# raulmur/ORB_SLAM

Measured on AMD Instinct MI355X. Metric: frames/s ORB extract+match @640x480, 1000 kp, higher is better.
Workload: dtype u8; 1 GPU; vga: 640x480 grayscale stream, 8 levels, nFeatures 1000, S-blocks frames, extract + Hamming top-2 match vs previous frame (BASELINE.json configs[1] + the frame-to-frame match of the metric); resident_frames_per_gpu=2048, lanes=4, parity_checked_frames=0, parity_mismatches=0, library_build_id=15f67f48a050b108, lane_placement=2

## Files before the change

orb_slam_amd/csrc/k_fast.hip:

```cpp
#include <algorithm>
#include <type_traits>

#include "orbx_device.h"
#include "orbx_launch.h"
#include "k_blur_strip.h"

namespace orbx {

__device__ __forceinline__ int fast_pair_test(const uint8_t* c, int S, int v, int t) {
    const int x0 = c[3 * S], x1 = c[3 * S + 1], x2 = c[2 * S + 2], x3 = c[S + 3], x4 = c[3], x5 = c[-S + 3], x6 = c[-2 * S + 2], x7 = c[-3 * S + 1];
    const int x8 = c[-3 * S], x9 = c[-3 * S - 1], x10 = c[-2 * S - 2], x11 = c[-S - 3], x12 = c[-3], x13 = c[S - 3], x14 = c[2 * S - 2], x15 = c[3 * S - 1];
    const int a = imax3(imax3(imin(x0, x8), imin(x1, x9), imin(x2, x10)), imax3(imin(x3, x11), imin(x4, x12), imin(x5, x13)), imax(imin(x6, x14), imin(x7, x15)));
    const int bq = imin3(imin3(imax(x0, x8), imax(x1, x9), imax(x2, x10)), imin3(imax(x3, x11), imax(x4, x12), imax(x5, x13)), imin(imax(x6, x14), imax(x7, x15)));
    return (int)(v - a > t) | (int)(bq - v > t);
}

__device__ __forceinline__ int fast_score_raw(const uint8_t* c, int S, int v, int tmin) {
    int x[16];
    x[0] = c[3 * S]; x[1] = c[3 * S + 1]; x[2] = c[2 * S + 2]; x[3] = c[S + 3]; x[4] = c[3]; x[5] = c[-S + 3]; x[6] = c[-2 * S + 2]; x[7] = c[-3 * S + 1];
    x[8] = c[-3 * S]; x[9] = c[-3 * S - 1]; x[10] = c[-2 * S - 2]; x[11] = c[-S - 3]; x[12] = c[-3]; x[13] = c[S - 3]; x[14] = c[2 * S - 2]; x[15] = c[3 * S - 1];
    int hi3[16], lo3[16];
#pragma unroll
    for (int k = 0; k < 16; k++) {
        hi3[k] = imax3(x[k], x[(k + 1) & 15], x[(k + 2) & 15]);
        lo3[k] = imin3(x[k], x[(k + 1) & 15], x[(k + 2) & 15]);
    }
    int hi9[16], lo9[16];
#pragma unroll
    for (int k = 0; k < 16; k++) {
        hi9[k] = imax3(hi3[k], hi3[(k + 3) & 15], hi3[(k + 6) & 15]);
        lo9[k] = imin3(lo3[k], lo3[(k + 3) & 15], lo3[(k + 6) & 15]);
    }
    const int min_hi9 = imin3(imin3(imin3(hi9[0], hi9[1], hi9[2]), imin3(hi9[3], hi9[4], hi9[5]), imin3(hi9[6], hi9[7], hi9[8])),
                              imin3(imin3(hi9[9], hi9[10], hi9[11]), imin3(hi9[12], hi9[13], hi9[14]), hi9[15]), 255);
    const int max_lo9 = imax3(imax3(imax3(lo9[0], lo9[1], lo9[2]), imax3(lo9[3], lo9[4], lo9[5]), imax3(lo9[6], lo9[7], lo9[8])),
                              imax3(imax3(lo9[9], lo9[10], lo9[11]), imax3(lo9[12], lo9[13], lo9[14]), lo9[15]), 0);
    const int s = imax(v - min_hi9, max_lo9 - v) - 1;
    return s >= tmin ? s : 0;
}

struct FastHdr { int n_hi, n_lo, overflow, pad1; int wsum[8]; int pad2[4]; };
static_assert(sizeof(FastHdr) == 64, "LDS carve");

__device__ __forceinline__ int lane_rank(unsigned long long m) {
    return (int)__builtin_amdgcn_mbcnt_hi((unsigned)(m >> 32), __builtin_amdgcn_mbcnt_lo((unsigned)m, 0u));
}
template <bool ALIGNED, int NT, int PPT, bool GATHER = false>
__device__ __forceinline__ void fast_band_task(const Batch& b, int frame, int item, uint8_t* smem) {
    constexpr int NW = NT / 64;
    static_assert((NW & (NW - 1)) == 0, "wave roles rotate modulo NW");
    constexpr int Q0CAP = fast_q0cap(PPT), Q1CAP = FAST_Q1CAP, Q2CAP = FAST_Q2CAP, Q3CAP = FAST_Q3CAP;
    constexpr int WQ_BYTES = fast_wave_queue_bytes(PPT);
    const DevGeom& g = b.g;
    const BandGeom bg = b.bands[item];
    const int level = bg.level;
    const LevelGeom& L = g.lv[level];
    const int lane = threadIdx.x & 63, wave = ORBX_FAST_ROTATE ? (wave_id() + item) & (NW - 1) : wave_id(), tid = wave * 64 + lane;
    const int cw = bg.x1 - bg.x0 + 1, ch = bg.ey1 - bg.ey0 + 1;
    CellState* cst = b.cstate + (long long)frame * g.nbands_total + item;
    const int hint = b.fallback_hint ? (int)((uint32_t)cst->thr >> 8) : 0;
    if (cw <= 0 || ch <= 0) {
        if (tid == 0) { CellState st; st.n_all = 0; st.n_hi = 0; st.n_lo = 0; st.thr = g.tmin; *cst = st; }
        return;
    }
    const int own_lo = bg.y0 - bg.ey0, own_hi = bg.y1 - bg.ey0;
    const int gxb = (bg.x0 - 3) & ~3;
    const int xoff = (bg.x0 - 3) - gxb;
    const int nd = fast_row_dwords(xoff, cw);
    const int S = nd * 4;
    const int x_first = xoff + 3;
    const int nrows = ch + 6;
    FastHdr* hdr = reinterpret_cast<FastHdr*>(smem);
    unsigned long long* cmask = reinterpret_cast<unsigned long long*>(smem + sizeof(FastHdr));
    uint8_t* wq = smem + sizeof(FastHdr) + g.fast_max_chunks * 8 + wave * WQ_BYTES;
    uint32_t* q0 = reinterpret_cast<uint32_t*>(wq);
    uint16_t* q1 = reinterpret_cast<uint16_t*>(wq + Q0CAP * 4);
    uint16_t* q2 = q1 + Q1CAP;
    uint16_t* q3 = q2 + Q2CAP;
    uint8_t* s_img = smem + sizeof(FastHdr) + g.fast_max_chunks * 8 + NW * WQ_BYTES;
    uint8_t* s_sc = s_img + g.fast_max_img;
    const int q_own_lo = (3 + own_lo) * S, q_own_hi = (3 + own_hi + 1) * S;
    const int nchunks = (q_own_hi - q_own_lo + 63) >> 6;
    long long stride64;
    const uint8_t* src = plain_plane<GATHER>(b, L, level, frame, stride64);
    auto clear_lds = [&]() {
        for (int i = tid; i < ((nrows * S + 15) >> 4); i += NT) reinterpret_cast<uint4*>(s_sc)[i] = make_uint4(0, 0, 0, 0);
        if (tid < (int)(sizeof(FastHdr) / 4)) reinterpret_cast<int*>(hdr)[tid] = 0;
        for (int i = tid; i < nchunks; i += NT) cmask[i] = 0ull;
    };
    if (ALIGNED) {
        typedef const void __attribute__((address_space(1))) * gptr_t;
        typedef void __attribute__((address_space(3))) * lptr_t;
        const uint8_t* src0 = src + (long long)(bg.ey0 - 3) * stride64 + gxb;
        clear_lds();
        {
            const int cpr = nd >> 2, nchunks16 = nrows * cpr;
            const float inv_cpr = bg.inv_cpr;
            for (int q0 = 64 * wave; q0 < nchunks16; q0 += 64 * NW) {
                const int q = q0 + lane;
                int r, c;
                split_px(imin(q, nchunks16 - 1), cpr, inv_cpr, r, c);
                const uint8_t* ga = src0 + (long long)r * stride64 + 16 * c;
                if (q < nchunks16) __builtin_amdgcn_global_load_lds((gptr_t)ga, (lptr_t)(s_img + 16 * q0), 16, 0, 0);
            }
        }
        asm volatile("s_waitcnt vmcnt(0)" ::: "memory");
    } else {
        const int total = nrows * nd;
        const float inv_nd0 = bg.inv_nd;
        const uint8_t* src0 = src + (long long)(bg.ey0 - 3) * stride64 + gxb;
        const int xm = L.w - 1 - gxb;
        for (int i0 = 0; i0 < total; i0 += NT * 8) {
            uint32_t v4[8];
#pragma unroll
            for (int k = 0; k < 8; k++) {
                const int i = i0 + k * NT + tid;
                v4[k] = 0;
                if (i < total) {
                    int r, d;
                    split_px(i, nd, inv_nd0, r, d);
                    const uint8_t* row = src0 + (long long)r * stride64;
                    v4[k] = (uint32_t)row[imin(4 * d, xm)] | (uint32_t)row[imin(4 * d + 1, xm)] << 8 | (uint32_t)row[imin(4 * d + 2, xm)] << 16 |
                            (uint32_t)row[imin(4 * d + 3, xm)] << 24;
                }
            }
            if (i0 == 0) clear_lds();
#pragma unroll
            for (int k = 0; k < 8; k++) {
                const int i = i0 + k * NT + tid;
                if (i < total) reinterpret_cast<uint32_t*>(s_img)[i] = v4[k];
            }
        }
    }
    __syncthreads();

    constexpr int FAST_HINT_RUN = 6;
    int tmin = ORBX_FAST_TWO_PASS ? (hint >= FAST_HINT_RUN && g.fast_th > 7 ? 7 : g.fast_th) : g.tmin;
    const float inv_nd = bg.inv_nd;
    int n0 = 0, n1 = 0, n2 = 0, n3 = 0;

    auto score_vals = [&](bool on, int p) {
        int sc = 0;
        if (on) {
            const uint8_t* c = s_img + p;
            sc = fast_score_raw(c, S, c[0], tmin);
            s_sc[p] = (uint8_t)sc;
        }
        const unsigned long long mk = __ballot(sc != 0);
        if (mk) {
            const int add = __popcll(mk);
            if (n3 + add <= Q3CAP) { if (sc) q3[n3 + lane_rank(mk)] = (uint16_t)p; }
            n3 += add;
        }
    };
    auto score_step = [&](const uint16_t* q, int m) { score_vals(lane < m, lane < m ? (int)q[lane] : 0); };
    auto pair_step = [&](const uint16_t* q, int m) {
        int pass = 0, p = 0;
        if (lane < m) {
            p = q[lane];
            const uint8_t* c = s_img + p;
            pass = fast_pair_test(c, S, c[0], tmin);
        }
        const unsigned long long mk = __ballot(pass);
        if (mk) {
            if (pass) q2[n2 + lane_rank(mk)] = (uint16_t)p;
            n2 += __popcll(mk);
            if (n2 >= 64) { n2 -= 64; score_step(q2 + n2, 64); }
        }
    };
    auto expand_step = [&](const uint32_t* q, int m) {
        uint32_t e = 0;
        if (lane < m) e = q[lane];
        const int idx = (int)(e & 0x3FFFu);
        int r, d;
        split_px(idx, nd, inv_nd, r, d);
        const int col0 = 4 * d - x_first;
        const int f[4] = {(int)((e >> 15) & 1u) & (int)((unsigned)col0 < (unsigned)cw), (int)((e >> 14) & 1u) & (int)((unsigned)(col0 + 1) < (unsigned)cw),
                          (int)((e >> 31) & 1u) & (int)((unsigned)(col0 + 2) < (unsigned)cw), (int)((e >> 30) & 1u) & (int)((unsigned)(col0 + 3) < (unsigned)cw)};
#pragma unroll
        for (int j = 0; j < 4; j++) {
            const unsigned long long mk = __ballot(f[j]);
            if (mk) {
                if (f[j]) q1[n1 + lane_rank(mk)] = (uint16_t)(4 * idx + j);
                n1 += __popcll(mk);
            }
            if (j & 1) while (n1 >= 64) { n1 -= 64; pair_step(q1 + n1, 64); }
        }
    };

    const uint32_t M8 = 0x00FF00FFu, HH = 0x80008000u;
    uint32_t KD = (uint32_t)(0x8000 - tmin - 1) * 0x00010001u;
    auto compass4 = [&](uint32_t C, uint32_t E, uint32_t W, uint32_t Nn, uint32_t Ss) -> uint32_t {
        uint32_t P[2];
#pragma unroll
        for (int hlf = 0; hlf < 2; hlf++) {
            const uint32_t c = hlf ? (C >> 8) & M8 : C & M8, n = hlf ? (Nn >> 8) & M8 : Nn & M8, s = hlf ? (Ss >> 8) & M8 : Ss & M8,
                           e = hlf ? (E >> 8) & M8 : E & M8, w = hlf ? (W >> 8) & M8 : W & M8;
            const uint32_t vd = c + KD, vb = KD - c;
            const uint32_t dk = ((vd - n) | (vd - s)) & ((vd - e) | (vd - w));
            const uint32_t br = ((n + vb) | (s + vb)) & ((e + vb) | (w + vb));
            P[hlf] = dk | br;
        }
        return (P[0] & HH) | ((P[1] & HH) >> 1);
    };
    const int i_begin = 3 * nd, i_end = (ch + 3) * nd;
    constexpr int RG = NW * 64 * PPT;
    auto round = [&](auto full_c, int base) {
        constexpr bool FULL = decltype(full_c)::value;
        const int i0 = base + wave * 64 + lane;
        uint32_t C[PPT], E[PPT], W[PPT], Nn[PPT], Ss[PPT];
#pragma unroll
        for (int k = 0; k < PPT; k++) {
            const int ik = FULL ? i0 + k * NW * 64 : imin(i0 + k * NW * 64, i_end - 1);
            const uint8_t* pk = s_img + 4 * ik;
            C[k] = *reinterpret_cast<const uint32_t*>(pk);
            E[k] = __builtin_amdgcn_alignbyte(*reinterpret_cast<const uint32_t*>(pk + 4), C[k], 3);
            W[k] = __builtin_amdgcn_alignbyte(C[k], *reinterpret_cast<const uint32_t*>(pk - 4), 1);
            Nn[k] = *reinterpret_cast<const uint32_t*>(pk - 3 * S);
            Ss[k] = *reinterpret_cast<const uint32_t*>(pk + 3 * S);
        }
#pragma unroll
        for (int k = 0; k < PPT; k++) {
            const int i = i0 + k * NW * 64;
            uint32_t Q = compass4(C[k], E[k], W[k], Nn[k], Ss[k]);
            if (!FULL && i >= i_end) Q = 0;
            const unsigned long long mk = __ballot(Q != 0);
            if (mk) {
                if (Q) q0[n0 + lane_rank(mk)] = Q | (uint32_t)i;
                n0 += __popcll(mk);
                if (n0 >= 64) { n0 -= 64; expand_step(q0 + n0, 64); }
            }
        }
    };
    for (;;) {
    {
        int base = i_begin;
        for (; base + RG <= i_end; base += RG) round(std::true_type{}, base);
        if (base < i_end) round(std::false_type{}, base);
    }
    if (n0) expand_step(q0, n0);
    for (int base = 0; base < n1 + n2; base += 64) {
        const int i = base + lane;
        const bool on = i < n1 + n2;
        score_vals(on, on ? (int)(i < n1 ? q1[i] : q2[i - n1]) : 0);
    }
    if (n3 > Q3CAP && lane == 0) hdr->overflow = 1;
    __syncthreads();

    auto nms_test = [&](int p, int s) -> bool {
        const uint8_t* sp = s_sc + p;
        const int mx = imax3(imax3(sp[-1], sp[1], sp[-S]), imax3(sp[S], sp[-S - 1], sp[-S + 1]), imax(sp[S - 1], sp[S + 1]));
        if (s > mx) {
            const int bit = p - q_own_lo;
            atomicOr(&cmask[bit >> 6], 1ull << (bit & 63));
        }
        return s > mx;
    };
    auto nms_px = [&](int p, int s) {
        if (nms_test(p, s)) {
            if (s >= g.fast_th) atomicAdd(&hdr->n_hi, 1);
            if (s >= 7) atomicAdd(&hdr->n_lo, 1);
        }
    };
    if (!hdr->overflow) {
        int c_hi = 0, c_lo = 0;
        for (int i0 = 0; i0 < n3; i0 += 64) {
            const int i = i0 + lane;
            int s = 0;
            bool keep = false;
            if (i < n3) {
                const int p = q3[i];
                s = s_sc[p];
                keep = p >= q_own_lo && p < q_own_hi && nms_test(p, s);
            }
            c_hi += __popcll(__ballot(keep && s >= g.fast_th));
            c_lo += __popcll(__ballot(keep && s >= 7));
        }
        if (lane == 0 && (c_hi | c_lo)) { atomicAdd(&hdr->n_hi, c_hi); atomicAdd(&hdr->n_lo, c_lo); }
    } else {
        const int d_lo = q_own_lo >> 2, d_hi = q_own_hi >> 2;
        for (int i = d_lo + tid; i < d_hi; i += NT) {
            uint32_t sc4 = reinterpret_cast<const uint32_t*>(s_sc)[i];
            while (sc4) {
                const int j = (__ffs((int)sc4) - 1) >> 3;
                const int s = (int)((sc4 >> (8 * j)) & 255u);
                sc4 &= ~(255u << (8 * j));
                nms_px(4 * i + j, s);
            }
        }
    }
    __syncthreads();
    if (tmin <= 7 || __builtin_amdgcn_readfirstlane(hdr->n_hi) > 3) break;
    __syncthreads();
    clear_lds();
    tmin = 7;
    KD = (uint32_t)(0x8000 - 7 - 1) * 0x00010001u;
    n0 = n1 = n2 = n3 = 0;
    __syncthreads();
    }
    Cand* out = b.cand + (long long)frame * g.frame_cands + L.cand_base + bg.cand_off;
    const float inv_S = bg.inv_s;
    int run_base = 0;
    for (int c0 = 0; c0 < nchunks; c0 += NT) {
        const bool busy = c0 + 64 * wave < nchunks;
        unsigned long long m = 0ull;
        int cnt = 0, incl = 0;
        if (busy) {
            if (c0 + tid < nchunks) m = cmask[c0 + tid];
            cnt = __popcll(m);
            incl = wave_scan_inclusive(cnt);
        }
        if (NW > 1) {
            if (lane == 63) hdr->wsum[wave] = incl;
            __syncthreads();
        }
        int run = run_base + incl - cnt, total = NW > 1 ? 0 : __builtin_amdgcn_readlane(incl, 63);
        if (NW > 1 && busy) {
#pragma unroll
            for (int wv = 0; wv < NW; wv++) { const int t = hdr->wsum[wv]; if (wv < wave) run += t; total += t; }
        }
        while (m) {
            const int bit = __ffsll((long long)m) - 1;
            m &= m - 1;
            const int p = q_own_lo + (c0 + tid) * 64 + bit;
            int r, xr;
            split_px(p, S, inv_S, r, xr);
            Cand e;
            e.pos = (uint32_t)(bg.x0 + xr - x_first) | ((uint32_t)(bg.ey0 + r - 3) << 16);
            e.resp = (float)s_sc[p];
            out[run++] = e;
        }
        run_base += total;
        if (NW > 1 && c0 + NT < nchunks) __syncthreads();
    }
    if (tid == 0) {
        CellState st;
        st.n_all = run_base; st.n_hi = hdr->n_hi; st.n_lo = hdr->n_lo;
        st.thr = tmin | ((st.n_hi <= 3 && g.fast_th > 7 ? imin(hint + 1, FAST_HINT_RUN) : 0) << 8);
        *cst = st;
    }
}

template <bool ALIGNED, int NT, int PPT, bool GATHER>
__device__ __forceinline__ void k_fast_cells_body(const Batch& b) {
    extern __shared__ __attribute__((aligned(16))) uint8_t smem[];
    int frame, item;
    if (!frame_item_magic(b, blockIdx.x, (unsigned)b.g.nbands_total, b.g.nbands_magic, frame, item)) return;
    fast_band_task<ALIGNED, NT, PPT, GATHER>(b, frame, item, smem);
}
template <bool ALIGNED, int NT, int PPT>
__global__ __launch_bounds__(NT) void k_fast_cells(Batch b) { k_fast_cells_body<ALIGNED, NT, PPT, false>(b); }
template <bool ALIGNED, int NT, int PPT>
__global__ __launch_bounds__(NT) void k_fast_cells_gather(Batch b) { k_fast_cells_body<ALIGNED, NT, PPT, true>(b); }

template <bool ALIGNED, bool SMALL, bool GATHER>
__device__ __forceinline__ void k_fast_blur_body(const Batch& b) {
    extern __shared__ __attribute__((aligned(16))) uint8_t smem[];
    constexpr FastShape A = SMALL ? FAST_SMALL : FAST_LARGE;
    constexpr int NW = A.threads / 64;
    const DevGeom& g = b.g;
    const int nblur = (g.nbtiles_total_s + NW - 1) / NW;
    const int per_frame = nblur + g.nbands_total;
    const int frame = blockIdx.x / per_frame, item = blockIdx.x - frame * per_frame;
    if (item < nblur) {
        const int t = item * NW + wave_id();
        if (t < g.nbtiles_total_s) blur_strip<ALIGNED, BLUR_ROWS_SMALL, GATHER>(b, frame, t);
    } else fast_band_task<ALIGNED, A.threads, A.ppt, GATHER>(b, frame, item - nblur, smem);
}
template <bool ALIGNED, bool SMALL>
__global__ __launch_bounds__(SMALL ? FAST_SMALL.threads : FAST_LARGE.threads) void k_fast_blur(Batch b) { k_fast_blur_body<ALIGNED, SMALL, false>(b); }
template <bool ALIGNED, bool SMALL>
__global__ __launch_bounds__(SMALL ? FAST_SMALL.threads : FAST_LARGE.threads) void k_fast_blur_gather(Batch b) { k_fast_blur_body<ALIGNED, SMALL, true>(b); }


int launch_fast(const Batch& b, const HostGeom& hg, hipStream_t stream, bool fuse_blur) {
    const DevGeom& g = hg.g;
    const int F = b.nframes;
    const bool aligned = (level0_bits(b) & 3) == 0;
    const size_t lds = (size_t)g.fast_lds_bytes;
    auto launch = [&](auto kern, int threads) -> bool {
        if (lds > 64 * 1024 && hipFuncSetAttribute(reinterpret_cast<const void*>(kern), hipFuncAttributeMaxDynamicSharedMemorySize, (int)lds) != hipSuccess) return false;
        hipLaunchKernelGGL(kern, dim3(frame_item_blocks(b, g.nbands_total)), dim3(threads), lds, stream, b);
        return true;
    };
    constexpr FastShape A = FAST_SMALL, B = FAST_LARGE;
    bool ok;
    if (fuse_blur) {
        const int threads = g.fast_small ? A.threads : B.threads;
        const int per_frame = (g.nbtiles_total_s + threads / 64 - 1) / (threads / 64) + g.nbands_total;
        auto launch2 = [&](auto kern) -> bool {
            if (lds > 64 * 1024 && hipFuncSetAttribute(reinterpret_cast<const void*>(kern), hipFuncAttributeMaxDynamicSharedMemorySize, (int)lds) != hipSuccess) return false;
            hipLaunchKernelGGL(kern, dim3(F * per_frame), dim3(threads), lds, stream, b);
            return true;
        };
        if (b.img_tab) {
            if (g.fast_small) ok = aligned ? launch2(k_fast_blur_gather<true, true>) : launch2(k_fast_blur_gather<false, true>);
            else ok = aligned ? launch2(k_fast_blur_gather<true, false>) : launch2(k_fast_blur_gather<false, false>);
        } else if (g.fast_small) ok = aligned ? launch2(k_fast_blur<true, true>) : launch2(k_fast_blur<false, true>);
        else ok = aligned ? launch2(k_fast_blur<true, false>) : launch2(k_fast_blur<false, false>);
    } else if (b.img_tab) {
        if (g.fast_small) ok = aligned ? launch(k_fast_cells_gather<true, A.threads, A.ppt>, A.threads) : launch(k_fast_cells_gather<false, A.threads, A.ppt>, A.threads);
        else ok = aligned ? launch(k_fast_cells_gather<true, B.threads, B.ppt>, B.threads) : launch(k_fast_cells_gather<false, B.threads, B.ppt>, B.threads);
    } else if (g.fast_small) ok = aligned ? launch(k_fast_cells<true, A.threads, A.ppt>, A.threads) : launch(k_fast_cells<false, A.threads, A.ppt>, A.threads);
    else ok = aligned ? launch(k_fast_cells<true, B.threads, B.ppt>, B.threads) : launch(k_fast_cells<false, B.threads, B.ppt>, B.threads);
    if (!ok) return ORBX_ERR_DEVICE;
    ORBX_LAUNCH_CHECK();
    return ORBX_OK;
}

}
```

orb_slam_amd/csrc/orbx_geometry.hip:

```cpp
#include <cfloat>
#include <climits>
#include <cmath>
#include <cstdlib>
#include <cstring>

#include "orbx_internal.h"

namespace orbx {

static inline int round_even(double v) { return (int)std::lrint(v); }
static inline int floor_int(double v) { int i = (int)v; return i - (i > v); }
static inline int ceil_int(double v) { int i = (int)v; return i + (i < v); }
static inline int16_t sat16(float v) {
    int iv = round_even(v);
    return (int16_t)(iv < SHRT_MIN ? SHRT_MIN : iv > SHRT_MAX ? SHRT_MAX : iv);
}
static inline int align_up(int v, int a) { return (v + a - 1) / a * a; }

static int build_geometry_band(const orbx_params& p, int w, int h, HostGeom& out, std::string& err, const int band_px, const FastShape& shape) {
    const int threads = shape.threads;
    const int nl = p.nlevels;
    if (nl < 1 || nl > MAX_LEVELS) { err = "nlevels out of range [1,16]"; return ORBX_ERR_ARG; }
    if (p.nfeatures < 1) { err = "nfeatures must be >= 1"; return ORBX_ERR_ARG; }
    if (!(p.scale_factor > 1.0f) || p.scale_factor > 2.5f) { err = "scale_factor must be in (1, 2.5]"; return ORBX_ERR_ARG; }
// ... 138 lines not shown
                        bg.inv_nd = 1.0f / (float)nd;
                        bg.inv_s = 1.0f / (float)(nd * 4);
                        bg.inv_cpr = 1.0f / (float)(nd >> 2);
                    }
                    cand_off += bg.cand_cap;
                    c.cand_cap += bg.cand_cap;
                    c.nbands++;
                    out.bands.push_back(bg);
                }
                out.cells.push_back(c);
            }
        cell_base += L.ncells;
        cand_base += cand_off;
        L.sel_base = sel_base;
        L.sel_cap = std::min(cand_off, L.ncells * L.nfeat_cell + L.ncells * L.ncells + L.ndesired + 64);
        sel_base += L.sel_cap;
        L.slot_base = slot_base;
        slot_base += L.ndesired;
        L.quad_base = quad_base;
        quad_base += (L.ndesired + 3) / 4;

        L.btiles_x = (L.w + 247) / 248;
        L.btiles_y = (L.h + BLUR_ROWS - 1) / BLUR_ROWS;
        L.btile_base = btile_base;
        btile_base += L.btiles_x * L.btiles_y;
        L.btiles_y_s = (L.h + BLUR_ROWS_SMALL - 1) / BLUR_ROWS_SMALL;
        L.btile_base_s = btile_base_s;
        btile_base_s += L.btiles_x * L.btiles_y_s;
        {
            const int nsteps = (L.h + 31) / 32;
            L.mb_strips = (L.w + 32 * MB_TILES - 1) / (32 * MB_TILES);
            L.mb_bands = (nsteps + MB_BAND_STEPS - 1) / MB_BAND_STEPS;
            L.mb_band_steps = (nsteps + L.mb_bands - 1) / L.mb_bands;
            L.mb_n = L.mb_strips * L.mb_bands;
        }
        L.mb_base = mb_base;
        mb_base += L.mb_n;

        if (l > 0) {
            const int sw = g.lv[l - 1].w, sh = g.lv[l - 1].h, dw = L.w, dh = L.h;
            if (sw > 32767 || sh > 32767) { err = "image too large"; return ORBX_ERR_ARG; }
            const double inv_x = (double)dw / sw, inv_y = (double)dh / sh;
            const double scale_x = 1. / inv_x, scale_y = 1. / inv_y;
            L.tabx_off = (int)out.tabx.size();
            L.taby_off = (int)out.taby.size();
            for (int dx = 0; dx < dw; dx++) {
                float fx = (float)((dx + 0.5) * scale_x - 0.5);
                int sx = floor_int(fx);
                fx -= sx;
                if (sx < 0) { fx = 0; sx = 0; }
                if (sx >= sw - 1) { fx = 0; sx = sw - 1; }
                ResizeX e;
                e.sx = (int16_t)sx;
                e.sx1 = (int16_t)std::min(sx + 1, sw - 1);
                e.a0 = sat16((1.f - fx) * 2048);
                e.a1 = sat16(fx * 2048);
                out.tabx.push_back(e);
            }
            for (int dy = 0; dy < dh; dy++) {
                float fy = (float)((dy + 0.5) * scale_y - 0.5);
                int sy = floor_int(fy);
                fy -= sy;
                ResizeY e;
                e.sy0 = (int16_t)std::min(std::max(sy, 0), sh - 1);
                e.sy1 = (int16_t)std::min(std::max(sy + 1, 0), sh - 1);
                e.b0 = sat16((1.f - fy) * 2048);
                e.b1 = sat16(fy * 2048);
                out.taby.push_back(e);
            }
            {
                const ResizeX* tx = out.tabx.data() + L.tabx_off;
                const ResizeY* ty = out.taby.data() + L.taby_off;
                int nd_max = 1, nr_max = 1;
                for (int bx0 = 0; bx0 < dw; bx0 += 256) {
                    const int bx1 = std::min(bx0 + 255, dw - 1);
                    nd_max = std::max(nd_max, ((tx[bx1].sx1 - (tx[bx0].sx & ~3)) >> 2) + 1);
                }
                for (int by0 = 0; by0 < dh; by0 += RZ_ROWS) {
                    const int by1 = std::min(by0 + RZ_ROWS - 1, dh - 1);
                    nr_max = std::max(nr_max, ty[by1].sy1 - ty[by0].sy0 + 1);
                }
                L.rz_pitch = 4 * nd_max + 8;
                L.rz_rows = nr_max;
                int span = 1;
                for (int x0 = 0; x0 < dw; x0 += 4) span = std::max(span, tx[std::min(x0 + 3, dw - 1)].sx1 - tx[x0].sx + 1);
                L.rz_window = span <= 8 ? 1 : 0;
                if (L.rz_pitch * L.rz_rows > 64 * 1024) { err = "resize tile does not fit the LDS"; return ORBX_ERR_CAPACITY; }
            }
        }
    }
    {
        constexpr int tile[2] = {ORBX_PYR_TILE};
        g.npyr_groups = 0;
        out.pyr_tab.clear();
        bool ok = scaleFactor <= 2.0 && nl > 1 && !getenv("ORBX_PYR_PER_LEVEL");
        int l0 = 0;
        while (ok && l0 < nl - 1) {
            if (g.npyr_groups == PYR_MAX_GROUPS) { ok = false; break; }
            PyrGroup pg;
            memset(&pg, 0, sizeof(pg));
            pg.l0 = l0;
            constexpr int depth_cfg[2] = {ORBX_PYR_DEPTH};
            pg.depth = std::min(std::min(l0 == 0 ? depth_cfg[0] : depth_cfg[1], PYR_MAX_DEPTH), nl - 1 - l0);
            const LevelGeom& LD = g.lv[l0 + pg.depth];
            pg.ntx = (LD.w + tile[0] - 1) / tile[0];
            pg.nty = (LD.h + tile[1] - 1) / tile[1];
            auto chain = [&](int n, int tsz, bool is_x, std::vector<int>& tab) {
                const int base = (int)tab.size();
                tab.resize(base + (size_t)(pg.depth + 1) * (n + 1) * 2);
                auto at = [&](int k, int i, int e) -> int& { return tab[base + ((size_t)k * (n + 1) + i) * 2 + e]; };
                const int dim_d = is_x ? LD.w : LD.h;
                for (int i = 0; i <= n; i++) { at(pg.depth, i, 0) = std::min(i * tsz, dim_d); at(pg.depth, i, 1) = std::min((i + 1) * tsz, dim_d) - 1; }
                at(pg.depth, n, 1) = dim_d;
                for (int k = pg.depth; k >= 1; k--) {
                    const LevelGeom& Lk = g.lv[l0 + k];
                    const LevelGeom& Ls = g.lv[l0 + k - 1];
                    const int dk = is_x ? Lk.w : Lk.h, ds = is_x ? Ls.w : Ls.h;
                    for (int i = 0; i <= n; i++) {
                        const int s0 = at(k, i, 0);
                        int src = ds;
                        if (s0 < dk) src = is_x ? (out.tabx[Lk.tabx_off + s0].sx & ~3) : out.taby[Lk.taby_off + s0].sy0;
                        at(k - 1, i, 0) = src;
                    }
                    for (int i = 0; i < n; i++) {
                        const int e0 = std::min(at(k, i, 1), dk - 1);
                        int need = is_x ? out.tabx[Lk.tabx_off + e0].sx1 : out.taby[Lk.taby_off + e0].sy1;
                        need = std::max(need, at(k - 1, i + 1, 0) - 1);
                        if (is_x) need = std::min(need | 3, ds - 1);
                        at(k - 1, i, 1) = std::max(need, at(k - 1, i, 0));
                    }
                    at(k - 1, n, 1) = ds;
                }
                return base;
            };
            pg.xtab = chain(pg.ntx, tile[0], true, out.pyr_tab);
            pg.ytab = chain(pg.nty, tile[1], false, out.pyr_tab);
            int off = 0;
            for (int k = 0; k < pg.depth; k++) {
                int maxw = 4, maxh = 1;
                for (int i = 0; i < pg.ntx; i++) maxw = std::max(maxw, out.pyr_tab[pg.xtab + ((size_t)k * (pg.ntx + 1) + i) * 2 + 1] - out.pyr_tab[pg.xtab + ((size_t)k * (pg.ntx + 1) + i) * 2] + 1);
                for (int i = 0; i < pg.nty; i++) maxh = std::max(maxh, out.pyr_tab[pg.ytab + ((size_t)k * (pg.nty + 1) + i) * 2 + 1] - out.pyr_tab[pg.ytab + ((size_t)k * (pg.nty + 1) + i) * 2] + 1);
                pg.pitch[k] = align_up(maxw, 4) + 4;
                pg.lds_off[k] = off;
                off += align_up(pg.pitch[k] * maxh, 16);
            }
            pg.lds_bytes = off;
            if (off > 64 * 1024) { ok = false; break; }
            g.pyr[g.npyr_groups++] = pg;
            l0 += pg.depth;
        }
        if (!ok) { g.npyr_groups = 0; out.pyr_tab.clear(); }
    }
    {
        int max_px = 0, max_img = 0, max_chunks = 0;
        for (const BandGeom& c : out.bands) {
            const int cw = c.x1 - c.x0 + 1, ch = c.ey1 - c.ey0 + 1;
            if (cw <= 0 || ch <= 0) continue;
            max_px = std::max(max_px, cw * ch);
            if (cw > shape.max_cw) { err = "grid cell wider than " + std::to_string(shape.max_cw) + " pixels"; return ORBX_ERR_CAPACITY; }
            const int nd = fast_row_dwords(3, cw);
            max_img = std::max(max_img, nd * 4 * (ch + 6));
            max_chunks = std::max(max_chunks, (nd * 4 * (c.y1 - c.y0 + 1) + 63) / 64);
        }
        if (max_px > 65535 || max_img > 65536) { err = "grid cell band larger than 64 KiB with its halo"; return ORBX_ERR_CAPACITY; }
        g.fast_max_img = align_up(std::max(max_img, 16), 16);
        g.fast_max_chunks = align_up(max_chunks + 1, 2);
        g.fast_lds_bytes = 64  + g.fast_max_chunks * 8 + (threads / 64) * fast_wave_queue_bytes(shape.ppt) + 2 * g.fast_max_img + 16;
        if (g.fast_lds_bytes > 160 * 1024) { err = "grid cell does not fit the 160 KiB LDS"; return ORBX_ERR_CAPACITY; }
    }
    {
        int max_cell = 1, max_level = 1;
        for (const CellGeom& c : out.cells) max_cell = std::max(max_cell, (int)c.cand_cap);
        for (int l = 0; l < nl; l++) max_level = std::max(max_level, g.lv[l].sel_cap);
        g.sel_lds_entries = std::min(std::max(max_cell, max_level), 2048);
        g.sel_lds_cell = align_up(g.sel_lds_entries * ((int)sizeof(Cand) + 4), 16);
        g.sel_lds_level = g.sel_lds_cell;
        if (g.sel_lds_cell > 160 * 1024 || g.sel_lds_level > 160 * 1024) { err = "keypoint list does not fit the 160 KiB LDS"; return ORBX_ERR_CAPACITY; }
    }
    for (int l = 0; l < MAX_LEVELS; l++) {
        const bool live = l < nl;
        g.cell_bases[l] = live ? g.lv[l].cell_base : INT_MAX;
        g.quad_bases[l] = live ? g.lv[l].quad_base : INT_MAX;
        g.btile_bases[l] = live ? g.lv[l].btile_base : INT_MAX;
        g.btile_bases_s[l] = live ? g.lv[l].btile_base_s : INT_MAX;
        g.mb_bases[l] = live ? g.lv[l].mb_base : INT_MAX;
    }
    g.ncells_total = cell_base;
    g.nbands_total = (int)out.bands.size();
    g.nbands_magic = g.nbands_total > 1 ? (uint32_t)((1ull << 32) / (unsigned)g.nbands_total) + 1u : 0u;
    g.nbtiles_total = btile_base;
    g.nbtiles_total_s = btile_base_s;
    g.nmb_total = mb_base;
    g.nslots = slot_base;
    g.nquads = quad_base;
    g.frame_plane_bytes = align_up(plane_off, 256);
    g.frame_cands = cand_base;
    g.frame_sel = sel_base;
    return ORBX_OK;
}


int build_geometry(const orbx_params& p, int w, int h, HostGeom& out, std::string& err) {
    constexpr int LDS_FOR_FOUR = (160 * 1024) / 4 - 64;
    const FastShape small = FAST_SMALL, large = FAST_LARGE;
    {
        HostGeom trial;
        std::string e2;
        if (build_geometry_band(p, w, h, trial, e2, small.band_px, small) == ORBX_OK) {
            int max_cell_px = 0;
            for (const CellGeom& c : trial.cells) max_cell_px = std::max(max_cell_px, (c.x1 - c.x0 + 1) * (c.y1 - c.y0 + 1));
            if (max_cell_px <= 12288) {
                out = trial;
                out.g.fast_threads = small.threads;
                out.g.fast_small = 1;
                err.clear();
                return ORBX_OK;
            }
        }
    }
    int rc = build_geometry_band(p, w, h, out, err, large.band_px, large);
    if (rc != ORBX_OK) return rc;
    out.g.fast_threads = large.threads;
    out.g.fast_small = 0;
    if (out.g.fast_lds_bytes <= LDS_FOR_FOUR) return rc;
    for (int band = large.band_px - 512; band >= 4096; band -= 512) {
        HostGeom trial;
        std::string e2;
        if (build_geometry_band(p, w, h, trial, e2, band, large) == ORBX_OK && trial.g.fast_lds_bytes <= LDS_FOR_FOUR) {
            out = trial;
            out.g.fast_threads = large.threads;
            out.g.fast_small = 0;
            err.clear();
            return ORBX_OK;
        }
    }
    return rc;
}

}
```

orb_slam_amd/csrc/orbx_internal.h:

```cpp
#pragma once
#include <hip/hip_runtime.h>
#include <stdint.h>
#include <string>
#include <vector>

#include "orbx.h"
#include "orbx_host.h"

namespace orbx {

constexpr int MAX_LEVELS = 16;
constexpr int EDGE = 16;
constexpr int HALF_PATCH = 15;

struct Cand {
    uint32_t pos;
    float resp;
};

struct ResizeX { int16_t sx, sx1, a0, a1; };
struct ResizeY { int16_t sy0, sy1, b0, b1; };

struct LevelGeom {
    int w, h;
    int stride;
    int plane_off;
    int gcols, grows;
    int cellW, cellH;
    int ncells;
    int nfeat_cell;
    int ndesired;
    int cell_base;
    int cand_base;
    int sel_base, sel_cap;
    int slot_base;
    int quad_base;
    int tabx_off, taby_off;
    int rz_window;
    int rz_pitch, rz_rows;
    int btile_base, btiles_x, btiles_y;
    int btile_base_s, btiles_y_s;
    int mb_base, mb_n;
    int mb_strips, mb_bands, mb_band_steps;
    int blur_wvec;
    int blur_sel_last, blur_sel_halo;
    float scale;
    float kp_size;
};

struct CellGeom {
    int16_t x0, y0, x1, y1;
    int32_t skipped;
    int32_t cand_off;
    int32_t cand_cap;
    int32_t band0, nbands;
};

#ifndef ORBX_BLUR_WAVES
#define ORBX_BLUR_WAVES 2
#endif
#ifndef ORBX_BLUR_ON_DEMAND_DEFAULT
#define ORBX_BLUR_ON_DEMAND_DEFAULT 1
#endif
#ifndef ORBX_OD_MIN_FRAMES_DEFAULT
#define ORBX_OD_MIN_FRAMES_DEFAULT 32
#endif
#ifndef ORBX_DESC_PACKED_PATTERN
#define ORBX_DESC_PACKED_PATTERN 1
#endif
#ifndef ORBX_DESC_WAVES
#define ORBX_DESC_WAVES 4
#endif
constexpr int BLUR_WAVES = ORBX_BLUR_WAVES;
constexpr int DESC_WAVES = ORBX_DESC_WAVES;
#ifndef ORBX_BLUR_ROWS
#define ORBX_BLUR_ROWS 32
#endif
#ifndef ORBX_RZ_ROWS
#define ORBX_RZ_ROWS 48
#endif
#ifndef ORBX_BLUR_MFMA
#define ORBX_BLUR_MFMA 1
#endif
#ifndef ORBX_MB_BAND_STEPS
#define ORBX_MB_BAND_STEPS 8
#endif
constexpr int MB_BAND_STEPS = ORBX_MB_BAND_STEPS;
constexpr int MB_MAX_WIDTH = 1024;
constexpr int MB_TILES = 2;
#ifndef ORBX_MB_WAVES
#define ORBX_MB_WAVES 4
#endif
constexpr int MB_WAVES = ORBX_MB_WAVES;
constexpr int BLUR_ROWS = ORBX_BLUR_ROWS;
constexpr int BLUR_ROWS_SMALL = 8;
constexpr int RZ_ROWS = ORBX_RZ_ROWS;
struct FastShape { int threads, ppt, band_px, max_cw; };
#ifndef ORBX_FS
#define ORBX_FS 256, 1, 8192, 500
#endif
#ifndef ORBX_FL
#define ORBX_FL 256, 2, 7168, 6500
#endif
constexpr FastShape FAST_SMALL = {ORBX_FS};
constexpr FastShape FAST_LARGE = {ORBX_FL};
#ifndef ORBX_FAST_TWO_PASS
#define ORBX_FAST_TWO_PASS 1
#endif
#ifndef ORBX_FAST_ROTATE
#define ORBX_FAST_ROTATE 1
#endif
constexpr int FAST_Q1CAP = 192, FAST_Q2CAP = 128, FAST_Q3CAP = 192;
constexpr int fast_q0cap(int) { return 128; }
constexpr int fast_wave_queue_bytes(int ppt) { return fast_q0cap(ppt) * 4 + FAST_Q1CAP * 2 + FAST_Q2CAP * 2 + FAST_Q3CAP * 2; }
__host__ __device__ constexpr int fast_row_dwords(int xoff, int cw) { return (((xoff + cw + 6 + 3) >> 2) + 3) & ~3; }
struct BandGeom {
    int16_t x0, x1;
    int16_t y0, y1;
    int16_t ey0, ey1;
    int32_t level;
    int32_t cand_off;
    int32_t cand_cap;
    float inv_nd, inv_s, inv_cpr;
};

constexpr int XCD_AFFINITY_MIN_FRAMES = 64;
#ifndef ORBX_PYR_DEPTH
#define ORBX_PYR_DEPTH 4, 4
#endif
constexpr int PYR_MAX_GROUPS = 4, PYR_MAX_DEPTH = 8;
struct PyrGroup {
    int l0, depth;
    int ntx, nty;
    int xtab, ytab;
    int lds_off[PYR_MAX_DEPTH];
    int pitch[PYR_MAX_DEPTH];
    int lds_bytes;
};
#ifndef ORBX_PYR_TILE
#define ORBX_PYR_TILE 16, 16
#endif

constexpr int QUOTA_LDS_PER_CELL = 10;
constexpr int QUOTA_MAX_CELLS = 160 * 1024 / QUOTA_LDS_PER_CELL / 64 * 64;
struct CellState { int32_t n_all, n_hi, n_lo, thr; };
struct CellSel { int32_t thr, nkeys, nretain, out_off; };

struct DevGeom {
    int nlevels;
    int ncells_total;
    int nbands_total;
    uint32_t nbands_magic;
    int nbtiles_total, nbtiles_total_s;
    int nmb_total;
    int nslots;
    int nquads;
    int quota_cells;
    int score_type, fast_th, tmin;
    int fp_contract;
    int frame_plane_bytes;
    int frame_cands;
    int frame_sel;
    int sel_lds_cell, sel_lds_level, sel_lds_entries;
    int fast_max_img, fast_max_chunks, fast_lds_bytes;
    int fast_threads;
    int fast_small;
    int npyr_groups;
    PyrGroup pyr[PYR_MAX_GROUPS];
    int umax[HALF_PATCH + 1];
    int cell_bases[MAX_LEVELS], quad_bases[MAX_LEVELS], btile_bases[MAX_LEVELS], btile_bases_s[MAX_LEVELS], mb_bases[MAX_LEVELS];
    LevelGeom lv[MAX_LEVELS];
};

struct ImgSrc {
    const uint8_t* data;
    long long row_stride;
};
static_assert(sizeof(ImgSrc) == 16, "one scalar dwordx4 per table entry");

struct Batch {
    DevGeom g;
    const CellGeom* cells;
    const BandGeom* bands;
    const ResizeX* tabx;
    const ResizeY* taby;
    const int* pyr_tab;
    const uint8_t* img;
    long long img_row_stride, img_frame_stride;
    uint8_t* pyr;
    uint8_t* blur;
    Cand* cand;
    Cand* sel;
    CellState* cstate;
    int fallback_hint;
    CellSel* csel;
    int32_t* level_total;
    int32_t* level_count;
    int32_t* status;
    int32_t* long_cells;
    orbx_keypoint* out_kps;
    uint8_t* out_desc;
    int32_t* out_n;
    int32_t* out_status;
    int cap;
    int nframes;
    int xcd_affinity;
    int od_min_frames;
    int blur_on_demand;
    const ImgSrc* img_tab;
    unsigned long long img_tab_bits;
    long long img_tab_min_stride;
};

static inline unsigned long long level0_bits(const Batch& b) {
    return b.img_tab ? b.img_tab_bits : ((uintptr_t)b.img | (unsigned long long)b.img_row_stride | (unsigned long long)b.img_frame_stride);
}
static inline long long level0_min_stride(const Batch& b) { return b.img_tab ? b.img_tab_min_stride : b.img_row_stride; }

struct ColorArgs {
    const uint8_t* src;
    long long src_row_stride, src_frame_stride;
    const ImgSrc* tab;
    unsigned long long tab_bits;
    uint8_t* dst;
    uint8_t* dst2;
    long long dst_row_stride, dst_frame_stride;
    int w, h;
    int f0;
    int cpr, items;
};
static inline int pix_channels(int fmt) {
    switch (fmt) {
        case ORBX_PIX_GRAY8: return 1;
        case ORBX_PIX_RGB8: case ORBX_PIX_BGR8: return 3;
        case ORBX_PIX_RGBA8: case ORBX_PIX_BGRA8: return 4;
        default: return 0;
    }
}
int launch_to_gray(const ColorArgs& a, int nframes, int fmt, hipStream_t stream);

struct HostGeom {
    DevGeom g;
    std::vector<CellGeom> cells;
    std::vector<BandGeom> bands;
    std::vector<ResizeX> tabx;
    std::vector<ResizeY> taby;
    std::vector<int> pyr_tab;
    std::vector<int> features_per_level;
    std::vector<float> scale, inv_scale;
};

int build_geometry(const orbx_params& p, int w, int h, HostGeom& out, std::string& err);

enum Stage { ST_PYRAMID = 0, ST_FAST_CELLS, ST_QUOTA, ST_CELL_SELECT, ST_LEVEL_SELECT, ST_BLUR, ST_DESCRIBE, ST_COUNT };

struct StageTimer {
    bool enabled = false;
    std::vector<hipEvent_t> pool;
    std::vector<int> pool_stage;
    double ms[ST_COUNT] = {0};
    long launches[ST_COUNT] = {0};
};

struct SideStream {
    Stream aux;
    Event fork, join;
};
int launch_extract(const Batch& b, const HostGeom& hg, hipStream_t stream, int stop_after, StageTimer* timer, const SideStream* side,
                   int phases = ORBX_PHASE_ALL);
bool describe_od_supported(const Batch& b, const HostGeom& hg);
int launch_describe_od(const Batch& b, const HostGeom& hg, hipStream_t stream);

}
```

Baseline: 449,600 frames/s.

## Use sparse score bitmask in FAST bands with dense sub-band fallback

By default the FAST band kernel now records detections as an LDS bitmask plus per-wave queued scores, instead of clearing and writing a full dense byte score plane. The scores are scattered back into the image buffer only for non-max suppression. If the queue overflows, the band is redone in two half-height dense sub-bands, and a per-band state bit makes later frames start in dense mode. This is meant to cut LDS clearing and score-plane traffic and to lower the LDS footprint. In exchange it adds atomics on the mask, extra sync points, and possible recomputation on dense bands.

```diff
diff --git a/orb_slam_amd/csrc/k_fast.hip b/orb_slam_amd/csrc/k_fast.hip
--- a/orb_slam_amd/csrc/k_fast.hip
+++ b/orb_slam_amd/csrc/k_fast.hip
@@ -39,30 +39,23 @@
     return s >= tmin ? s : 0;
 }
 
-struct FastHdr { int n_hi, n_lo, overflow, pad1; int wsum[8]; int pad2[4]; };
+struct FastHdr { int n_hi, n_lo, overflow, n_scored; int wsum[8]; int pad2[4]; };
 static_assert(sizeof(FastHdr) == 64, "LDS carve");
+constexpr int FAST_PASS_OK = 0, FAST_PASS_RETRY = 1, FAST_PASS_OVERFLOW = 2;
+constexpr int FAST_DENSE_MARK = 1 << 16;
 
 __device__ __forceinline__ int lane_rank(unsigned long long m) {
     return (int)__builtin_amdgcn_mbcnt_hi((unsigned)(m >> 32), __builtin_amdgcn_mbcnt_lo((unsigned)m, 0u));
 }
-template <bool ALIGNED, int NT, int PPT, bool GATHER = false>
-__device__ __forceinline__ void fast_band_task(const Batch& b, int frame, int item, uint8_t* smem) {
+template <bool ALIGNED, int NT, int PPT, bool GATHER, bool DENSE>
+__device__ __forceinline__ int fast_band_pass(const Batch& b, const LevelGeom& L, const uint8_t* src, long long stride64, const BandGeom& bg, int wave, int lane,
+                                              uint8_t* smem, int tmin, bool retry_ok, bool lds_in_use, Cand* out, int& n_list, int& n_hi, int& n_lo, int& n_scored) {
     constexpr int NW = NT / 64;
-    static_assert((NW & (NW - 1)) == 0, "wave roles rotate modulo NW");
     constexpr int Q0CAP = fast_q0cap(PPT), Q1CAP = FAST_Q1CAP, Q2CAP = FAST_Q2CAP, Q3CAP = FAST_Q3CAP;
     constexpr int WQ_BYTES = fast_wave_queue_bytes(PPT);
     const DevGeom& g = b.g;
-    const BandGeom bg = b.bands[item];
-    const int level = bg.level;
-    const LevelGeom& L = g.lv[level];
-    const int lane = threadIdx.x & 63, wave = ORBX_FAST_ROTATE ? (wave_id() + item) & (NW - 1) : wave_id(), tid = wave * 64 + lane;
+    const int tid = wave * 64 + lane;
     const int cw = bg.x1 - bg.x0 + 1, ch = bg.ey1 - bg.ey0 + 1;
-    CellState* cst = b.cstate + (long long)frame * g.nbands_total + item;
-    const int hint = b.fallback_hint ? (int)((uint32_t)cst->thr >> 8) : 0;
-    if (cw <= 0 || ch <= 0) {
-        if (tid == 0) { CellState st; st.n_all = 0; st.n_hi = 0; st.n_lo = 0; st.thr = g.tmin; *cst = st; }
-        return;
-    }
     const int own_lo = bg.y0 - bg.ey0, own_hi = bg.y1 - bg.ey0;
     const int gxb = (bg.x0 - 3) & ~3;
     const int xoff = (bg.x0 - 3) - gxb;
@@ -77,17 +70,19 @@
     uint16_t* q1 = reinterpret_cast<uint16_t*>(wq + Q0CAP * 4);
     uint16_t* q2 = q1 + Q1CAP;
     uint16_t* q3 = q2 + Q2CAP;
+    uint8_t* q3s = reinterpret_cast<uint8_t*>(q3 + Q3CAP);
     uint8_t* s_img = smem + sizeof(FastHdr) + g.fast_max_chunks * 8 + NW * WQ_BYTES;
-    uint8_t* s_sc = s_img + g.fast_max_img;
+    uint8_t* s_sc = s_img + g.fast_sub_img;
+    uint32_t* s_m = reinterpret_cast<uint32_t*>(s_img + g.fast_max_img);
     const int q_own_lo = (3 + own_lo) * S, q_own_hi = (3 + own_hi + 1) * S;
     const int nchunks = (q_own_hi - q_own_lo + 63) >> 6;
-    long long stride64;
-    const uint8_t* src = plain_plane<GATHER>(b, L, level, frame, stride64);
     auto clear_lds = [&]() {
-        for (int i = tid; i < ((nrows * S + 15) >> 4); i += NT) reinterpret_cast<uint4*>(s_sc)[i] = make_uint4(0, 0, 0, 0);
+        if (DENSE) for (int i = tid; i < ((nrows * S + 15) >> 4); i += NT) reinterpret_cast<uint4*>(s_sc)[i] = make_uint4(0, 0, 0, 0);
+        else for (int i = tid; i < (((nrows * S) >> 5) + 5) >> 2; i += NT) reinterpret_cast<uint4*>(s_m)[i] = make_uint4(0, 0, 0, 0);
         if (tid < (int)(sizeof(FastHdr) / 4)) reinterpret_cast<int*>(hdr)[tid] = 0;
         for (int i = tid; i < nchunks; i += NT) cmask[i] = 0ull;
     };
+    if (lds_in_use) __syncthreads();
     if (ALIGNED) {
         typedef const void __attribute__((address_space(1))) * gptr_t;
         typedef void __attribute__((address_space(3))) * lptr_t;
@@ -134,8 +129,6 @@
     }
     __syncthreads();
 
-    constexpr int FAST_HINT_RUN = 6;
-    int tmin = ORBX_FAST_TWO_PASS ? (hint >= FAST_HINT_RUN && g.fast_th > 7 ? 7 : g.fast_th) : g.tmin;
     const float inv_nd = bg.inv_nd;
     int n0 = 0, n1 = 0, n2 = 0, n3 = 0;
 
@@ -144,12 +137,19 @@
         if (on) {
             const uint8_t* c = s_img + p;
             sc = fast_score_raw(c, S, c[0], tmin);
-            s_sc[p] = (uint8_t)sc;
+            if (DENSE) s_sc[p] = (uint8_t)sc;
+            else if (sc) atomicOr(&s_m[p >> 5], 1u << (p & 31));
         }
         const unsigned long long mk = __ballot(sc != 0);
         if (mk) {
             const int add = __popcll(mk);
-            if (n3 + add <= Q3CAP) { if (sc) q3[n3 + lane_rank(mk)] = (uint16_t)p; }
+            if (n3 + add <= Q3CAP) {
+                if (sc) {
+                    const int at = n3 + lane_rank(mk);
+                    q3[at] = (uint16_t)p;
+                    if (!DENSE) q3s[at] = (uint8_t)sc;
+                }
+            }
             n3 += add;
         }
     };
@@ -189,7 +189,7 @@
     };
 
     const uint32_t M8 = 0x00FF00FFu, HH = 0x80008000u;
-    uint32_t KD = (uint32_t)(0x8000 - tmin - 1) * 0x00010001u;
+    const uint32_t KD = (uint32_t)(0x8000 - tmin - 1) * 0x00010001u;
     auto compass4 = [&](uint32_t C, uint32_t E, uint32_t W, uint32_t Nn, uint32_t Ss) -> uint32_t {
         uint32_t P[2];
 #pragma unroll
@@ -232,7 +232,6 @@
             }
         }
     };
-    for (;;) {
     {
         int base = i_begin;
         for (; base + RG <= i_end; base += RG) round(std::true_type{}, base);
@@ -245,11 +244,29 @@
         score_vals(on, on ? (int)(i < n1 ? q1[i] : q2[i - n1]) : 0);
     }
     if (n3 > Q3CAP && lane == 0) hdr->overflow = 1;
+    if (DENSE && n3 && lane == 0) atomicAdd(&hdr->n_scored, n3);
     __syncthreads();
+    const int overflow = __builtin_amdgcn_readfirstlane(hdr->overflow);
+    if (!DENSE) {
+        if (overflow) return FAST_PASS_OVERFLOW;
+        for (int i = lane; i < n3; i += 64) s_img[q3[i]] = q3s[i];
+        __syncthreads();
+    }
 
     auto nms_test = [&](int p, int s) -> bool {
-        const uint8_t* sp = s_sc + p;
-        const int mx = imax3(imax3(sp[-1], sp[1], sp[-S]), imax3(sp[S], sp[-S - 1], sp[-S + 1]), imax(sp[S - 1], sp[S + 1]));
+        int mx;
+        if (DENSE) {
+            const uint8_t* sp = s_sc + p;
+            mx = imax3(imax3(sp[-1], sp[1], sp[-S]), imax3(sp[S], sp[-S - 1], sp[-S + 1]), imax(sp[S - 1], sp[S + 1]));
+        } else {
+            const uint8_t* sp = s_img + p;
+            auto bits3 = [&](int o) -> uint32_t { return __builtin_amdgcn_alignbit(s_m[(o >> 5) + 1], s_m[o >> 5], (uint32_t)(o & 31)); };
+            const uint32_t mu = bits3(p - S - 1), mc = bits3(p - 1), md = bits3(p + S - 1);
+            const int u0 = mu & 1u ? sp[-S - 1] : 0, u1 = mu & 2u ? sp[-S] : 0, u2 = mu & 4u ? sp[-S + 1] : 0;
+            const int c0 = mc & 1u ? sp[-1] : 0, c2 = mc & 4u ? sp[1] : 0;
+            const int d0 = md & 1u ? sp[S - 1] : 0, d1 = md & 2u ? sp[S] : 0, d2 = md & 4u ? sp[S + 1] : 0;
+            mx = imax3(imax3(c0, c2, u1), imax3(d1, u0, u2), imax(d0, d2));
+        }
         if (s > mx) {
             const int bit = p - q_own_lo;
             atomicOr(&cmask[bit >> 6], 1ull << (bit & 63));
@@ -262,7 +279,7 @@
             if (s >= 7) atomicAdd(&hdr->n_lo, 1);
         }
     };
-    if (!hdr->overflow) {
+    if (!DENSE || !overflow) {
         int c_hi = 0, c_lo = 0;
         for (int i0 = 0; i0 < n3; i0 += 64) {
             const int i = i0 + lane;
@@ -270,7 +287,7 @@
             bool keep = false;
             if (i < n3) {
                 const int p = q3[i];
-                s = s_sc[p];
+                s = DENSE ? s_sc[p] : q3s[i];
                 keep = p >= q_own_lo && p < q_own_hi && nms_test(p, s);
             }
             c_hi += __popcll(__ballot(keep && s >= g.fast_th));
@@ -290,17 +307,14 @@
         }
     }
     __syncthreads();
-    if (tmin <= 7 || __builtin_amdgcn_readfirstlane(hdr->n_hi) > 3) break;
-    __syncthreads();
-    clear_lds();
-    tmin = 7;
-    KD = (uint32_t)(0x8000 - 7 - 1) * 0x00010001u;
-    n0 = n1 = n2 = n3 = 0;
-    __syncthreads();
-    }
-    Cand* out = b.cand + (long long)frame * g.frame_cands + L.cand_base + bg.cand_off;
+    const int pass_hi = __builtin_amdgcn_readfirstlane(hdr->n_hi), pass_lo = __builtin_amdgcn_readfirstlane(hdr->n_lo);
+    if (retry_ok && tmin > 7 && pass_hi <= 3) return FAST_PASS_RETRY;
+    n_hi += pass_hi;
+    n_lo += pass_lo;
+    if (DENSE) n_scored += __builtin_amdgcn_readfirstlane(hdr->n_scored);
+    const uint8_t* s_val = DENSE ? s_sc : s_img;
     const float inv_S = bg.inv_s;
-    int run_base = 0;
+    int run_base = n_list;
     for (int c0 = 0; c0 < nchunks; c0 += NT) {
         const bool busy = c0 + 64 * wave < nchunks;
         unsigned long long m = 0ull;
@@ -327,16 +341,68 @@
             split_px(p, S, inv_S, r, xr);
             Cand e;
             e.pos = (uint32_t)(bg.x0 + xr - x_first) | ((uint32_t)(bg.ey0 + r - 3) << 16);
-            e.resp = (float)s_sc[p];
+            e.resp = (float)s_val[p];
             out[run++] = e;
         }
         run_base += total;
         if (NW > 1 && c0 + NT < nchunks) __syncthreads();
     }
+    n_list = run_base;
+    return FAST_PASS_OK;
+}
+
+template <bool ALIGNED, int NT, int PPT, bool GATHER = false>
+__device__ __forceinline__ void fast_band_task(const Batch& b, int frame, int item, uint8_t* smem) {
+    constexpr int NW = NT / 64;
+    static_assert((NW & (NW - 1)) == 0, "wave roles rotate modulo NW");
+    const DevGeom& g = b.g;
+    const BandGeom bg = b.bands[item];
+    const int level = bg.level;
+    const LevelGeom& L = g.lv[level];
+    const int lane = threadIdx.x & 63, wave = ORBX_FAST_ROTATE ? (wave_id() + item) & (NW - 1) : wave_id(), tid = wave * 64 + lane;
+    CellState* cst = b.cstate + (long long)frame * g.nbands_total + item;
+    const uint32_t left = (uint32_t)cst->thr;
+    const int hint = b.fallback_hint ? (int)((left >> 8) & 0xFFu) : 0;
+    if (bg.x1 - bg.x0 + 1 <= 0 || bg.ey1 - bg.ey0 + 1 <= 0) {
+        if (tid == 0) { CellState st; st.n_all = 0; st.n_hi = 0; st.n_lo = 0; st.thr = g.tmin; *cst = st; }
+        return;
+    }
+    long long stride64;
+    const uint8_t* src = plain_plane<GATHER>(b, L, level, frame, stride64);
+    Cand* out = b.cand + (long long)frame * g.frame_cands + L.cand_base + bg.cand_off;
+
+    constexpr int FAST_HINT_RUN = 6;
+    int tmin = ORBX_FAST_TWO_PASS ? (hint >= FAST_HINT_RUN && g.fast_th > 7 ? 7 : g.fast_th) : g.tmin;
+    int n_list = 0, n_hi = 0, n_lo = 0, n_scored = 0;
+    bool dense = (left & (uint32_t)FAST_DENSE_MARK) != 0, used = false;
+    if (!dense) {
+        int rc = fast_band_pass<ALIGNED, NT, PPT, GATHER, false>(b, L, src, stride64, bg, wave, lane, smem, tmin, true, false, out, n_list, n_hi, n_lo, n_scored);
+        if (rc == FAST_PASS_RETRY) {
+            tmin = 7;
+            rc = fast_band_pass<ALIGNED, NT, PPT, GATHER, false>(b, L, src, stride64, bg, wave, lane, smem, tmin, false, true, out, n_list, n_hi, n_lo, n_scored);
+        }
+        dense = rc == FAST_PASS_OVERFLOW;
+        used = true;
+    }
+    int mark = 0;
+    if (dense) {
+        for (;;) {
+            n_list = n_hi = n_lo = n_scored = 0;
+            for (int k = 0; k < 2; k++) {
+                BandGeom sub = bg;
+                if (!fast_sub_band(bg, k, sub)) break;
+                fast_band_pass<ALIGNED, NT, PPT, GATHER, true>(b, L, src, stride64, sub, wave, lane, smem, tmin, false, used, out, n_list, n_hi, n_lo, n_scored);
+                used = true;
+            }
+            if (tmin <= 7 || n_hi > 3) break;
+            tmin = 7;
+        }
+        if (n_scored > 2 * FAST_Q3CAP) mark = FAST_DENSE_MARK;
+    }
     if (tid == 0) {
         CellState st;
-        st.n_all = run_base; st.n_hi = hdr->n_hi; st.n_lo = hdr->n_lo;
-        st.thr = tmin | ((st.n_hi <= 3 && g.fast_th > 7 ? imin(hint + 1, FAST_HINT_RUN) : 0) << 8);
+        st.n_all = n_list; st.n_hi = n_hi; st.n_lo = n_lo;
+        st.thr = tmin | ((n_hi <= 3 && g.fast_th > 7 ? imin(hint + 1, FAST_HINT_RUN) : 0) << 8) | mark;
         *cst = st;
     }
 }
diff --git a/orb_slam_amd/csrc/orbx_geometry.hip b/orb_slam_amd/csrc/orbx_geometry.hip
--- a/orb_slam_amd/csrc/orbx_geometry.hip
+++ b/orb_slam_amd/csrc/orbx_geometry.hip
@@ -314,7 +314,7 @@
         if (!ok) { g.npyr_groups = 0; out.pyr_tab.clear(); }
     }
     {
-        int max_px = 0, max_img = 0, max_chunks = 0;
+        int max_px = 0, max_img = 0, max_chunks = 0, max_sub = 0;
         for (const BandGeom& c : out.bands) {
             const int cw = c.x1 - c.x0 + 1, ch = c.ey1 - c.ey0 + 1;
             if (cw <= 0 || ch <= 0) continue;
@@ -323,11 +323,17 @@
             const int nd = fast_row_dwords(3, cw);
             max_img = std::max(max_img, nd * 4 * (ch + 6));
             max_chunks = std::max(max_chunks, (nd * 4 * (c.y1 - c.y0 + 1) + 63) / 64);
+            for (int k = 0; k < 2; k++) {
+                BandGeom sub = c;
+                if (fast_sub_band(c, k, sub)) max_sub = std::max(max_sub, nd * 4 * (sub.ey1 - sub.ey0 + 1 + 6));
+            }
         }
         if (max_px > 65535 || max_img > 65536) { err = "grid cell band larger than 64 KiB with its halo"; return ORBX_ERR_CAPACITY; }
         g.fast_max_img = align_up(std::max(max_img, 16), 16);
         g.fast_max_chunks = align_up(max_chunks + 1, 2);
-        g.fast_lds_bytes = 64  + g.fast_max_chunks * 8 + (threads / 64) * fast_wave_queue_bytes(shape.ppt) + 2 * g.fast_max_img + 16;
+        g.fast_sub_img = align_up(std::max(max_sub, 16), 16);
+        const int area = std::max(g.fast_max_img + align_up(((g.fast_max_img >> 5) + 2) * 4, 16), 2 * g.fast_sub_img);
+        g.fast_lds_bytes = 64  + g.fast_max_chunks * 8 + (threads / 64) * fast_wave_queue_bytes(shape.ppt) + area + 16;
         if (g.fast_lds_bytes > 160 * 1024) { err = "grid cell does not fit the 160 KiB LDS"; return ORBX_ERR_CAPACITY; }
     }
     {
diff --git a/orb_slam_amd/csrc/orbx_internal.h b/orb_slam_amd/csrc/orbx_internal.h
--- a/orb_slam_amd/csrc/orbx_internal.h
+++ b/orb_slam_amd/csrc/orbx_internal.h
@@ -112,7 +112,7 @@
 #endif
 constexpr int FAST_Q1CAP = 192, FAST_Q2CAP = 128, FAST_Q3CAP = 192;
 constexpr int fast_q0cap(int) { return 128; }
-constexpr int fast_wave_queue_bytes(int ppt) { return fast_q0cap(ppt) * 4 + FAST_Q1CAP * 2 + FAST_Q2CAP * 2 + FAST_Q3CAP * 2; }
+constexpr int fast_wave_queue_bytes(int ppt) { return fast_q0cap(ppt) * 4 + FAST_Q1CAP * 2 + FAST_Q2CAP * 2 + FAST_Q3CAP * 3; }
 __host__ __device__ constexpr int fast_row_dwords(int xoff, int cw) { return (((xoff + cw + 6 + 3) >> 2) + 3) & ~3; }
 struct BandGeom {
     int16_t x0, x1;
@@ -123,6 +123,19 @@
     int32_t cand_cap;
     float inv_nd, inv_s, inv_cpr;
 };
+
+__host__ __device__ inline bool fast_sub_band(const BandGeom& bg, int k, BandGeom& sub) {
+    const int n = bg.y1 - bg.y0 + 1, h0 = (n + 1) >> 1;
+    if (k == 0) {
+        sub.y1 = (int16_t)(bg.y0 + h0 - 1);
+        if (n > h0) sub.ey1 = (int16_t)(sub.y1 + 1);
+        return true;
+    }
+    if (n <= h0) return false;
+    sub.y0 = (int16_t)(bg.y0 + h0);
+    sub.ey0 = (int16_t)(sub.y0 - 1);
+    return true;
+}
 
 constexpr int XCD_AFFINITY_MIN_FRAMES = 64;
 #ifndef ORBX_PYR_DEPTH
@@ -163,6 +176,7 @@
     int frame_sel;
     int sel_lds_cell, sel_lds_level, sel_lds_entries;
     int fast_max_img, fast_max_chunks, fast_lds_bytes;
+    int fast_sub_img;
     int fast_threads;
     int fast_small;
     int npyr_groups;
```

Result: slower. 430,200 frames/s (-4.3%).
